# lpiccinelli-eth/UniDepth

Measured on NVIDIA H100. Metric: images/sec UniDepthV2.infer ViT-L/14 480x640, higher is better.
Workload: dtype f16 operands, f32 accumulate/residual

## Files before the change

unidepth_b200/csrc/gemm.cu:

```cuda
#include "common.h"
#include "ptx.cuh"

namespace udb {

constexpr int BM = 128;
constexpr int BK = 64;
constexpr int kEpiWarps = 8;
constexpr int kTP = 36;
constexpr int kThreads = (kEpiWarps + 4) * 32;

struct GemmArgs {
  int M, N, K, num_kb;
  int tiles_m, tiles_n;
  int a_mode;
  int conv_B, conv_H, conv_W, conv_cpb , conv_off, conv_TH, conv_TW, conv_tx, conv_ty;
  const float* bias;
  const float* gamma;
  const void* resid;
  int resid_f32;
  void* out;
  int out_f32;
  __half* out2;
  int out2_leaky;
  int act;
  int store_mode;
  long long ldc, ldr;
  int rpg, gstride, roff;
  int resid_mod, resid_roff;
  int ct_k, ct_cout, ct_h, ct_w, ct_pad;
  int conv_coff;
  const float* head_w;
  float head_b, head_add;
  int a_wrap;
  int out_split;
  float* stats_out;
  const float* ln_stats;
  const float* ln_c1;
  int ln_parts, ln_part_cols;
  float ln_eps;
};

template <int BN>
struct GemmCfg {
  static constexpr int kStages = BN >= 256 ? 3 : (BN >= 192 ? 4 : (BN >= 128 ? 5 : 7));
  static constexpr int kABytes = BM * BK * 2;
  static constexpr int kBBytes = BN * BK * 2;
  static constexpr int kStageBytes = kABytes + kBBytes;
  static constexpr int kStagingBytes = kEpiWarps * (32 * kTP * 4 + 2 * 32 * 4);
  static constexpr int kSmemBytes = kStages * kStageBytes + kStagingBytes + 256 ;
  static_assert(kSmemBytes <= 232448, "shared memory per block");
};

struct EpiWarp {
  float* T;
  float* Twg;
  uint32_t* roff_out;
  uint32_t* roff_res;
  int wg, wq, grp, lane, r_in_tile;
};

template <int BN, bool LNF>
__device__ __forceinline__ void epilogue_tile(const GemmArgs& p, const EpiWarp& w, const float (&acc)[BN / 2], const int mt,
                                              const int nt) {
  constexpr int kGroups = BN >= 64 ? 2 : 1;
  constexpr int kColsPerGrp = BN / kGroups;
  const int grp = w.grp, lane = w.lane, r_in_tile = w.r_in_tile;
  const bool active = grp < kGroups;
  float* T = w.T;
  uint32_t* roff_out = w.roff_out;
  uint32_t* roff_res = w.roff_res;
  bool valid = false;
  long long out_off = 0, res_off = 0;
  uint32_t vmask = 0;
  float ln_mean = 0.f, ln_rstd = 1.f;
  float st_pivot = 0.f, st_s1 = 0.f, st_s2 = 0.f;
  bool st_first = true;
  if (active) {

    const int m = mt * BM + r_in_tile;
    if (p.store_mode == UDB_STORE_CONVTILE || p.store_mode == UDB_STORE_HEAD) {
      const int per_img = p.conv_tx * p.conv_ty;
      const int b = mt / per_img;
      const int r = mt % per_img;
      const int y = (r / p.conv_tx) * p.conv_TH + r_in_tile / p.conv_TW;
      const int x = (r % p.conv_tx) * p.conv_TW + r_in_tile % p.conv_TW;
      valid = (b < p.conv_B) && (y < p.conv_H) && (x < p.conv_W);
      out_off = (((long long)b * p.conv_H + y) * p.conv_W + x) * p.ldc;
      res_off = (((long long)b * p.conv_H + y) * p.conv_W + x) * p.ldr;
    } else if (p.store_mode == UDB_STORE_CONVT) {
      valid = m < p.M;
      const int hw = p.ct_h * p.ct_w;
      const int b = m / hw;
      const int r = m % hw;
      const int y = r / p.ct_w, x = r % p.ct_w;
      const long long W2 = (long long)p.ct_w * p.ct_k + 2 * p.ct_pad;
      const long long H2 = (long long)p.ct_h * p.ct_k + 2 * p.ct_pad;
      out_off = ((b * H2 + (long long)y * p.ct_k + p.ct_pad) * W2 + (long long)x * p.ct_k + p.ct_pad) * p.ct_cout;
      res_off = out_off;
    } else {
      valid = m < p.M;
      long long orow = m;
      if (p.rpg > 0) orow = (long long)(m / p.rpg) * p.gstride + (m % p.rpg) + p.roff;
      out_off = orow * p.ldc;
      res_off = (p.resid_mod > 0) ? ((long long)(m % p.resid_mod) + p.resid_roff) * p.ldr
                                  : orow * p.ldr;
    }
    vmask = __ballot_sync(0xffffffffu, valid);
    roff_out[lane] = static_cast<uint32_t>(out_off);
    roff_res[lane] = static_cast<uint32_t>(res_off);
    __syncwarp();
    if (LNF && p.ln_stats) {
      const float2* sp = reinterpret_cast<const float2*>(p.ln_stats) + (long long)(valid ? m : 0) * p.ln_parts;
      float ms = 0.f, m2 = 0.f;
      for (int q = 0; q < p.ln_parts; ++q) ms += sp[q].x;
      ln_mean = ms / (float)p.ln_parts;
      for (int q = 0; q < p.ln_parts; ++q) {
        const float2 t = sp[q];
        m2 += t.y + (float)p.ln_part_cols * (t.x - ln_mean) * (t.x - ln_mean);
      }
      ln_rstd = rsqrtf(m2 / (float)(p.ln_parts * p.ln_part_cols) + p.ln_eps);
    }
  }
  const int frow = 16 * (w.wq & 1) + (lane >> 2), fcol = 2 * (lane & 3);
#pragma unroll
  for (int c = 0; c < kColsPerGrp; c += 32) {
    bar_sync(1 + w.wg, 128);
#pragma unroll
    for (int gi = 0; gi < kGroups; ++gi) {
      float* Tt = w.Twg + ((w.wq >> 1) | (gi << 1)) * 32 * kTP;
#pragma unroll
      for (int j = 0; j < 4; ++j) {
        const int f = ((gi * kColsPerGrp + c) / 8 + j) * 4;
        *reinterpret_cast<float2*>(Tt + frow * kTP + 8 * j + fcol) = make_float2(acc[f], acc[f + 1]);
        *reinterpret_cast<float2*>(Tt + (frow + 8) * kTP + 8 * j + fcol) = make_float2(acc[f + 2], acc[f + 3]);
      }
    }
    bar_sync(1 + w.wg, 128);
    if (!active) continue;
    const int col = grp * kColsPerGrp + c;
    const int n0 = nt * BN + col;
    float v[32];
#pragma unroll
    for (int j = 0; j < 32; j += 4) {
      const float4 t = *reinterpret_cast<const float4*>(T + lane * kTP + j);
      v[j] = t.x; v[j + 1] = t.y; v[j + 2] = t.z; v[j + 3] = t.w;
    }
    __syncwarp();
    if (n0 >= p.N) continue;
    if (LNF && p.ln_stats) {
      const float4* cp = reinterpret_cast<const float4*>(p.ln_c1 + n0);
      const float mr = ln_mean * ln_rstd;
#pragma unroll
      for (int j = 0; j < 8; ++j) {
        const float4 c4 = __ldg(cp + j);
        v[4 * j] = fmaf(v[4 * j], ln_rstd, -mr * c4.x);
        v[4 * j + 1] = fmaf(v[4 * j + 1], ln_rstd, -mr * c4.y);
        v[4 * j + 2] = fmaf(v[4 * j + 2], ln_rstd, -mr * c4.z);
        v[4 * j + 3] = fmaf(v[4 * j + 3], ln_rstd, -mr * c4.w);
      }
    }
    if (p.bias) {
      const float4* bp = reinterpret_cast<const float4*>(p.bias + n0);
#pragma unroll
      for (int j = 0; j < 8; ++j) {
        const float4 b4 = __ldg(bp + j);
        v[4 * j] += b4.x; v[4 * j + 1] += b4.y; v[4 * j + 2] += b4.z; v[4 * j + 3] += b4.w;
      }
    }
    if (p.act == UDB_ACT_GELU) {
#pragma unroll
      for (int j = 0; j < 32; j += 2) gelu_erf_pair(v[j], v[j + 1]);
    } else if (p.act == UDB_ACT_LEAKY) {
#pragma unroll
      for (int j = 0; j < 32; ++j) v[j] = leaky(v[j]);
    }
    if (p.store_mode == UDB_STORE_HEAD) {
      float head = p.head_b;
#pragma unroll
      for (int j = 0; j < 32; ++j) head = fmaf(v[j], __ldg(p.head_w + j), head);
      head = fminf(fmaxf(head, -8.0f), 8.0f) + p.head_add;
      if (valid) reinterpret_cast<float*>(p.out)[out_off] = expf(head);
      continue;
    }
    if (p.gamma) {
      const float4* gp = reinterpret_cast<const float4*>(p.gamma + n0);
#pragma unroll
      for (int j = 0; j < 8; ++j) {
        const float4 g4 = __ldg(gp + j);
        v[4 * j] *= g4.x; v[4 * j + 1] *= g4.y; v[4 * j + 2] *= g4.z; v[4 * j + 3] *= g4.w;
      }
    }
    long long coff = n0;
    if (p.store_mode == UDB_STORE_CONVT) {
      const int tap = n0 / p.ct_cout;
      const int co = n0 % p.ct_cout;
      const long long W2 = (long long)p.ct_w * p.ct_k + 2 * p.ct_pad;
      coff = ((long long)(tap / p.ct_k) * W2 + (tap % p.ct_k)) * p.ct_cout + co;
    }
    const uint32_t c32 = static_cast<uint32_t>(coff);
    const int l4 = (lane & 7) * 4, rq = lane >> 3;
    float* Trow = T + lane * kTP;
    auto stage_rows = [&](const float (&x)[32]) {
#pragma unroll
      for (int j = 0; j < 32; j += 4)
        *reinterpret_cast<float4*>(Trow + j) = make_float4(x[j], x[j + 1], x[j + 2], x[j + 3]);
    };
    auto for_rows = [&](auto&& body) {
      if (vmask == 0xffffffffu) {
#pragma unroll
        for (int i = 0; i < 8; ++i) body(4 * i + rq, true);
      } else {
#pragma unroll
        for (int i = 0; i < 8; ++i) body(4 * i + rq, ((vmask >> (4 * i + rq)) & 1u) != 0);
      }
    };
    if (p.resid) {
      if (p.resid_f32) {
        const float* rp = reinterpret_cast<const float*>(p.resid) + c32 + l4;
        float4 tmp[8];
        int k = 0;
        for_rows([&](int rr, bool ok) {
          tmp[k++] = ok ? *reinterpret_cast<const float4*>(rp + roff_res[rr]) : make_float4(0.f, 0.f, 0.f, 0.f);
        });
#pragma unroll
        for (int i = 0; i < 8; ++i) *reinterpret_cast<float4*>(T + (4 * i + rq) * kTP + l4) = tmp[i];
      } else {
        const __half* rp = reinterpret_cast<const __half*>(p.resid) + c32 + l4;
        uint2 tmp[8];
        int k = 0;
        for_rows([&](int rr, bool ok) {
          tmp[k++] = ok ? *reinterpret_cast<const uint2*>(rp + roff_res[rr]) : make_uint2(0u, 0u);
        });
#pragma unroll
        for (int i = 0; i < 8; ++i) {
          const float2 a = __half22float2(*reinterpret_cast<const __half2*>(&tmp[i].x));
          const float2 b = __half22float2(*reinterpret_cast<const __half2*>(&tmp[i].y));
          *reinterpret_cast<float4*>(T + (4 * i + rq) * kTP + l4) = make_float4(a.x, a.y, b.x, b.y);
        }
      }
      __syncwarp();
#pragma unroll
      for (int j = 0; j < 32; j += 4) {
        const float4 t = *reinterpret_cast<const float4*>(Trow + j);
        v[j] += t.x; v[j + 1] += t.y; v[j + 2] += t.z; v[j + 3] += t.w;
      }
      __syncwarp();
    }
    if (LNF && p.stats_out) {
      if (st_first) { st_pivot = v[0]; st_first = false; }
#pragma unroll
      for (int j = 0; j < 32; ++j) {
        const float dlt = v[j] - st_pivot;
        st_s1 += dlt;
        st_s2 = fmaf(dlt, dlt, st_s2);
      }
    }
    if (p.out) {
      stage_rows(v);
      __syncwarp();
      if (p.out_f32) {
        float* op = reinterpret_cast<float*>(p.out) + c32 + l4;
        for_rows([&](int rr, bool ok) {
          if (ok) *reinterpret_cast<float4*>(op + roff_out[rr]) = *reinterpret_cast<const float4*>(T + rr * kTP + l4);
        });
      } else {
        __half* op = reinterpret_cast<__half*>(p.out) + c32 + l4;
        if (p.out_split == 0) {
          for_rows([&](int rr, bool ok) {
            const float4 t = *reinterpret_cast<const float4*>(T + rr * kTP + l4);
            if (ok) *reinterpret_cast<uint2*>(op + roff_out[rr]) = make_uint2(pack_half2(t.x, t.y), pack_half2(t.z, t.w));
          });
        } else {
          for_rows([&](int rr, bool ok) {
            const float4 t = *reinterpret_cast<const float4*>(T + rr * kTP + l4);
            const uint2 hi = make_uint2(pack_half2(t.x, t.y), pack_half2(t.z, t.w));
            const float2 h01 = __half22float2(*reinterpret_cast<const __half2*>(&hi.x));
            const float2 h23 = __half22float2(*reinterpret_cast<const __half2*>(&hi.y));
            if (ok) {
              *reinterpret_cast<uint2*>(op + roff_out[rr]) = hi;
              *reinterpret_cast<uint2*>(op + roff_out[rr] + p.out_split) =
                  make_uint2(pack_half2(t.x - h01.x, t.y - h01.y), pack_half2(t.z - h23.x, t.w - h23.y));
            }
          });
        }
      }
      __syncwarp();
    }
    if (p.out2) {
      if (p.out2_leaky) {
#pragma unroll
        for (int j = 0; j < 32; ++j) v[j] = leaky(v[j]);
        stage_rows(v);
      } else if (!p.out) {
        stage_rows(v);
      }
      __syncwarp();
      __half* op = p.out2 + c32 + l4;
      for_rows([&](int rr, bool ok) {
        const float4 t = *reinterpret_cast<const float4*>(T + rr * kTP + l4);
        if (ok) *reinterpret_cast<uint2*>(op + roff_out[rr]) = make_uint2(pack_half2(t.x, t.y), pack_half2(t.z, t.w));
      });
      __syncwarp();
    }
  }
  if (LNF && p.stats_out && active && valid && !st_first) {
    const float n = (float)kColsPerGrp;
    const float mean_p = st_pivot + st_s1 / n;
    const float m2_p = fmaxf(st_s2 - st_s1 * st_s1 / n, 0.f);
    const long long orow = out_off / p.ldc;
    reinterpret_cast<float2*>(p.stats_out)[orow * (p.tiles_n * kGroups) + nt * kGroups + grp] = make_float2(mean_p, m2_p);
  }
}

template <int BN, bool LNF>
__global__ void __launch_bounds__(kThreads, 1)
gemm_f16_kernel(const __grid_constant__ CUtensorMap tmA, const __grid_constant__ CUtensorMap tmB,
                const GemmArgs p) {
  using Cfg = GemmCfg<BN>;
  constexpr int kStages = Cfg::kStages;
  extern __shared__ __align__(1024) uint8_t smem[];
  uint8_t* sA = smem;
  uint8_t* sB = smem + kStages * Cfg::kABytes;
  uint8_t* staging = smem + kStages * Cfg::kStageBytes;
  uint64_t* bars = reinterpret_cast<uint64_t*>(staging + Cfg::kStagingBytes);
  uint64_t* full_bar = bars;
  uint64_t* empty_bar = bars + kStages;

  const int warp = threadIdx.x >> 5;
  const int lane = threadIdx.x & 31;
  pdl_launch_dependents();

  if (threadIdx.x == 0) {
    if (smem_u32(smem) & 1023) __trap();
    prefetch_tmap(&tmA);
    prefetch_tmap(&tmB);
    for (int i = 0; i < kStages; ++i) {
      mbar_init(&full_bar[i], 1);
      mbar_init(&empty_bar[i], kEpiWarps);
    }
    fence_barrier_init();
  }
  __syncthreads();
  pdl_wait();

  const int num_tiles = p.tiles_m * p.tiles_n;

  if (warp >= kEpiWarps) {
    setmaxnreg_dec<40>();
    if (warp != kEpiWarps) return;
    const bool elected = elect_one();
    int stage = 0;
    uint32_t phase = 0;
    for (int tile = blockIdx.x; tile < num_tiles; tile += gridDim.x) {
      const int mt = tile / p.tiles_n;
      const int nt = tile % p.tiles_n;
      int cb = 0, cy = 0, cx = 0;
      if (p.a_mode == UDB_A_CONV3X3) {
        const int per_img = p.conv_tx * p.conv_ty;
        cb = mt / per_img;
        const int r = mt % per_img;
        cy = (r / p.conv_tx) * p.conv_TH + p.conv_off;
        cx = (r % p.conv_tx) * p.conv_TW + p.conv_off;
      }
      for (int kb = 0; kb < p.num_kb; ++kb) {
        mbar_wait(&empty_bar[stage], phase ^ 1);
        if (elected) {
          mbar_arrive_expect_tx(&full_bar[stage], Cfg::kStageBytes);
          if (p.a_mode == UDB_A_CONV3X3) {
            const int tap = kb / p.conv_cpb;
            const int c0 = p.conv_coff + (kb % p.conv_cpb) * BK;
            tma_load_4d(sA + stage * Cfg::kABytes, &tmA, &full_bar[stage], c0, cx + tap % 3, cy + tap / 3, cb);
          } else {
            int ka = kb * BK;
            if (p.a_wrap && ka >= p.a_wrap) ka -= p.a_wrap;
            tma_load_2d(sA + stage * Cfg::kABytes, &tmA, &full_bar[stage], ka, mt * BM);
          }
          tma_load_2d(sB + stage * Cfg::kBBytes, &tmB, &full_bar[stage], kb * BK, nt * BN);
        }
        __syncwarp();
        if (++stage == kStages) {
          stage = 0;
          phase ^= 1;
        }
      }
    }
  } else {
    setmaxnreg_inc<232>();
    const int wg = warp >> 2, wq = warp & 3;
    float* Twg = reinterpret_cast<float*>(staging) + wg * 4 * 32 * kTP;
    uint32_t* roff = reinterpret_cast<uint32_t*>(staging + kEpiWarps * 32 * kTP * 4) + warp * 64;
    const EpiWarp ctx{Twg + wq * 32 * kTP, Twg, roff, roff + 32, wg, wq, wq >> 1, lane, 64 * wg + 32 * (wq & 1) + lane};
    float acc[BN / 2];
#pragma unroll
    for (int i = 0; i < BN / 2; ++i) acc[i] = 0.f;
    int stage = 0;
    uint32_t phase = 0;
    for (int tile = blockIdx.x; tile < num_tiles; tile += gridDim.x) {
      const int mt = tile / p.tiles_n;
      const int nt = tile % p.tiles_n;
      int prev = -1;
      for (int kb = 0; kb < p.num_kb; ++kb) {
        mbar_wait(&full_bar[stage], phase);
        const uint64_t da = gmma_desc_sw128(smem_u32(sA + stage * Cfg::kABytes + wg * 64 * 128), 16, 1024);
        const uint64_t db = gmma_desc_sw128(smem_u32(sB + stage * Cfg::kBBytes), 16, 1024);
        wgmma_fence();
#pragma unroll
        for (int k = 0; k < BK / 16; ++k) WgmmaSS<BN>::run(acc, da + 2 * k, db + 2 * k, (kb | k) != 0 ? 1u : 0u);
        wgmma_commit();
        wgmma_wait<1>();
        if (prev >= 0 && lane == 0) mbar_arrive(&empty_bar[prev]);
        prev = stage;
        if (++stage == kStages) {
          stage = 0;
          phase ^= 1;
        }
      }
      wgmma_wait<0>();
      wgmma_fence_regs(acc);
      if (prev >= 0 && lane == 0) mbar_arrive(&empty_bar[prev]);
      epilogue_tile<BN, LNF>(p, ctx, acc, mt, nt);
    }
  }
}

template <int BN, bool LNF>
static int launch_gemm(const CUtensorMap& tmA, const CUtensorMap& tmB, const GemmArgs& a, cudaStream_t st) {
  using Cfg = GemmCfg<BN>;
  static std::atomic<uint64_t> attr_mask{0};
  if (first_on_device(attr_mask)) {
    cudaError_t e = cudaFuncSetAttribute(gemm_f16_kernel<BN, LNF>, cudaFuncAttributeMaxDynamicSharedMemorySize,
                                         Cfg::kSmemBytes);
    if (e != cudaSuccess) {
      set_error("gemm: cudaFuncSetAttribute(%d B smem): %s", Cfg::kSmemBytes, cudaGetErrorString(e));
      return 1;
    }
  }
  const int tiles = a.tiles_m * a.tiles_n;
  const int grid = tiles < num_sms() ? tiles : num_sms();
  cudaError_t e = launch_ex(gemm_f16_kernel<BN, LNF>, dim3(grid), dim3(kThreads), Cfg::kSmemBytes, st, 1, tmA, tmB, a);
  if (e != cudaSuccess) {
    set_error("gemm_f16_kernel launch: %s", cudaGetErrorString(e));
    return 1;
  }
  return check_launch("gemm_f16_kernel");
}

static bool aligned(const void* p, uintptr_t bytes) { return (reinterpret_cast<uintptr_t>(p) & (bytes - 1)) == 0; }

static int check_gemm_layout(const udb_gemm_t* g) {
  const int sm = g->store_mode;
  if (g->M < 1 || g->N < 1 || g->K < 1) { set_error("udb_gemm_f16: M=%d N=%d K=%d must be >= 1", g->M, g->N, g->K); return 1; }
  if (sm < UDB_STORE_ROWS || sm > UDB_STORE_HEAD) { set_error("udb_gemm_f16: unknown store_mode %d", sm); return 1; }
  const long long ldr = g->ldr > 0 ? g->ldr : g->ldc;
  if (sm == UDB_STORE_HEAD) {
    if (!g->out || !g->out_f32 || !aligned(g->out, 4)) { set_error("udb_gemm_f16: HEAD store needs a 4-byte aligned f32 `out`"); return 1; }
    if (!g->head_w || !aligned(g->head_w, 16)) { set_error("udb_gemm_f16: `head_w` must be non-null and 16-byte aligned"); return 1; }
  } else {
    if (g->out && !aligned(g->out, g->out_f32 ? 16 : 8)) {
      set_error("udb_gemm_f16: `out` %p must be %d-byte aligned", g->out, g->out_f32 ? 16 : 8); return 1;
    }
    if (g->out2 && !aligned(g->out2, 8)) { set_error("udb_gemm_f16: `out2` %p must be 8-byte aligned", g->out2); return 1; }
    if (g->resid && !aligned(g->resid, g->resid_f32 ? 16 : 8)) {
      set_error("udb_gemm_f16: `resid` %p must be %d-byte aligned", g->resid, g->resid_f32 ? 16 : 8); return 1;
    }
    if (sm != UDB_STORE_CONVT) {
      if ((g->out || g->out2) && (g->ldc < 1 || g->ldc % 4)) { set_error("udb_gemm_f16: `ldc`=%lld must be a positive multiple of 4", (long long)g->ldc); return 1; }
      if (g->resid && (ldr < 1 || ldr % 4)) { set_error("udb_gemm_f16: `ldr`=%lld must be a positive multiple of 4", ldr); return 1; }
      if ((g->out || g->out2) && g->ldc < (long long)g->N + g->out_split) {
        set_error("udb_gemm_f16: `ldc`=%lld < N + out_split = %lld: rows would overlap", (long long)g->ldc, (long long)g->N + g->out_split);
        return 1;
      }
      if (g->resid && ldr < g->N) { set_error("udb_gemm_f16: `ldr`=%lld < N=%d: residual rows would overlap", ldr, g->N); return 1; }
    }
  }
  if (g->out_split < 0 || g->out_split % 4) { set_error("udb_gemm_f16: `out_split`=%d must be a non-negative multiple of 4", g->out_split); return 1; }
  if (!aligned(g->bias, 16)) { set_error("udb_gemm_f16: `bias` %p must be 16-byte aligned", (const void*)g->bias); return 1; }
  if (!aligned(g->gamma, 16)) { set_error("udb_gemm_f16: `gamma` %p must be 16-byte aligned", (const void*)g->gamma); return 1; }
  if (!aligned(g->ln_c1, 16)) { set_error("udb_gemm_f16: `ln_c1` %p must be 16-byte aligned", (const void*)g->ln_c1); return 1; }
  if (!aligned(g->ln_stats_out, 8) || !aligned(g->ln_stats_in, 8)) { set_error("udb_gemm_f16: `ln_stats_*` must be 8-byte aligned"); return 1; }

  long long out_row = 0, res_row = 0;
  if (sm == UDB_STORE_ROWS) {
    const int m = g->M - 1;
    long long orow = m;
    if (g->rows_per_group > 0) {
      if (g->group_stride < 0 || g->row_offset < 0) {
        set_error("udb_gemm_f16: `group_stride`=%d and `row_offset`=%d must be >= 0", g->group_stride, g->row_offset); return 1;
      }
      const long long rpg = g->rows_per_group, grp = m / rpg;
      orow = grp * g->group_stride + m % rpg + g->row_offset;
      if (grp > 0 && (grp - 1) * g->group_stride + rpg - 1 + g->row_offset > orow) orow = (grp - 1) * g->group_stride + rpg - 1 + g->row_offset;
    }
    long long rrow = orow;
    if (g->resid_mod > 0) {
      if (g->resid_row_offset < 0) { set_error("udb_gemm_f16: `resid_row_offset`=%d must be >= 0", g->resid_row_offset); return 1; }
      rrow = (long long)(g->resid_mod < g->M ? g->resid_mod : g->M) - 1 + g->resid_row_offset;
    }
    out_row = orow * g->ldc;
    res_row = rrow * ldr;
  } else if (sm == UDB_STORE_CONVT) {
    if (g->ct_k < 1 || g->ct_h < 1 || g->ct_w < 1 || g->ct_pad < 0 || g->ct_cout < 1) {
      set_error("udb_gemm_f16: CONVT geometry `ct_k`=%d `ct_h`=%d `ct_w`=%d `ct_pad`=%d `ct_cout`=%d", g->ct_k, g->ct_h, g->ct_w, g->ct_pad,
                g->ct_cout);
      return 1;
    }
    if (g->N != g->ct_k * g->ct_k * g->ct_cout) { set_error("udb_gemm_f16: CONVT needs N == ct_k^2 * ct_cout (N=%d)", g->N); return 1; }
    const long long m = g->M - 1, hw = (long long)g->ct_h * g->ct_w, b = m / hw, r = m % hw, y = r / g->ct_w, x = r % g->ct_w;
    const long long W2 = (long long)g->ct_w * g->ct_k + 2 * g->ct_pad, H2 = (long long)g->ct_h * g->ct_k + 2 * g->ct_pad;
    out_row = res_row = ((b * H2 + y * g->ct_k + g->ct_pad) * W2 + x * g->ct_k + g->ct_pad) * g->ct_cout;
  } else {
    if (g->conv_B < 1 || g->conv_H < 1 || g->conv_W < 1) {
      set_error("udb_gemm_f16: conv_B=%d conv_H=%d conv_W=%d must be >= 1", g->conv_B, g->conv_H, g->conv_W); return 1;
    }
    const long long last_px = (long long)g->conv_B * g->conv_H * g->conv_W - 1;
    out_row = last_px * g->ldc;
    res_row = last_px * ldr;
  }
  const long long lim = 1ll << 32;
  if ((g->out || g->out2) && out_row >= lim) { set_error("udb_gemm_f16: `out` row offset %lld exceeds 2^32 elements", out_row); return 1; }
  if (g->resid && res_row >= lim) { set_error("udb_gemm_f16: `resid` row offset %lld exceeds 2^32 elements", res_row); return 1; }

  if (g->a_mode == UDB_A_CONV3X3) {
    const int pad = g->conv_off == 0 ? 2 : (g->conv_off == -1 ? 0 : -1);
    if (pad < 0) { set_error("udb_gemm_f16: `conv_off`=%d must be 0 (prepadded) or -1 (zero padding)", g->conv_off); return 1; }
    if (g->conv_inH != g->conv_H + pad || g->conv_inW != g->conv_W + pad) {
      set_error("udb_gemm_f16: `conv_inH`x`conv_inW` = %dx%d must be %dx%d for conv_off %d", g->conv_inH, g->conv_inW, g->conv_H + pad,
                g->conv_W + pad, g->conv_off);
      return 1;
    }
  }
  return 0;
}

}

extern "C" int udb_gemm_f16(const udb_gemm_t* g, void* stream) {
  using namespace udb;
  if (!g || !g->a || !g->w) { set_error("udb_gemm_f16: null operand"); return 1; }
  if (g->N % 32 != 0) { set_error("udb_gemm_f16: N=%d must be a multiple of 32", g->N); return 1; }
  if (check_gemm_layout(g)) return 1;
  GemmArgs a{};
  a.M = g->M; a.N = g->N; a.K = g->K;
  a.num_kb = (g->K + BK - 1) / BK;
  a.a_mode = g->a_mode;
  a.bias = g->bias; a.gamma = g->gamma; a.resid = g->resid; a.resid_f32 = g->resid_f32;
  a.out = g->out; a.out_f32 = g->out_f32; a.out2 = reinterpret_cast<__half*>(g->out2); a.out2_leaky = g->out2_leaky;
  a.act = g->act; a.store_mode = g->store_mode;
  a.ldc = g->ldc; a.ldr = g->ldr > 0 ? g->ldr : g->ldc;
  a.rpg = g->rows_per_group; a.gstride = g->group_stride; a.roff = g->row_offset;
  a.resid_mod = g->resid_mod; a.resid_roff = g->resid_row_offset;
  a.ct_k = g->ct_k; a.ct_cout = g->ct_cout; a.ct_h = g->ct_h; a.ct_w = g->ct_w; a.ct_pad = g->ct_pad;
  a.conv_coff = g->conv_coff;
  a.head_w = g->head_w; a.head_b = g->head_b; a.head_add = g->head_add;
  a.a_wrap = 0;
  a.out_split = g->out_split;
  if (g->a_split_k > 0) {
    if (g->a_mode != UDB_A_MATRIX || g->a_split_k % BK || g->K != 3 * g->a_split_k || g->lda < 2 * g->a_split_k) {
      set_error("udb_gemm_f16: split operands need a_mode MATRIX, K1 %% 64 == 0, K == 3*K1, lda >= 2*K1 (K1=%d K=%d lda=%d)",
                g->a_split_k, g->K, g->lda);
      return 1;
    }
    a.a_wrap = 2 * g->a_split_k;
  }
  a.stats_out = g->ln_stats_out; a.ln_stats = g->ln_stats_in; a.ln_c1 = g->ln_c1; a.ln_eps = g->ln_eps;
  a.ln_parts = g->ln_parts; a.ln_part_cols = g->ln_part_cols;
  if ((g->ln_stats_out || g->ln_stats_in) && g->store_mode != UDB_STORE_ROWS) {
    set_error("udb_gemm_f16: fused LayerNorm statistics need the ROWS store"); return 1;
  }
  if (g->ln_stats_in && (!g->ln_c1 || g->ln_parts <= 0 || g->ln_part_cols <= 0 || g->rows_per_group > 0)) {
    set_error("udb_gemm_f16: ln_stats_in needs ln_c1, ln_parts, ln_part_cols and an identity row map"); return 1;
  }
  if (g->out_split && (g->out_f32 || !g->out || g->store_mode != UDB_STORE_ROWS)) {
    set_error("udb_gemm_f16: out_split needs an f16 `out` with the ROWS store"); return 1;
  }

  int bn;
  if (g->store_mode == UDB_STORE_HEAD) {
    if (g->N != 32) { set_error("udb_gemm_f16: HEAD store needs N == 32"); return 1; }
    bn = 32;
  } else if (g->N % 256 == 0) bn = 256;
  else if (g->N % 192 == 0) bn = 192;
  else if (g->N % 128 == 0) bn = 128;
  else if (g->N % 64 == 0) bn = 64;
  else bn = 32;
  if (g->store_mode == UDB_STORE_CONVT && (g->ct_cout % 32) != 0) {
    set_error("udb_gemm_f16: CONVT needs Cout %% 32 == 0"); return 1;
  }
  a.tiles_n = (g->N + bn - 1) / bn;
  if (g->ln_stats_out) {
    const int groups = bn >= 64 ? 2 : 1;
    if (g->N % bn || g->ln_parts != a.tiles_n * groups || g->ln_part_cols != bn / groups) {
      set_error("udb_gemm_f16: ln_stats_out with N=%d runs as %d parts of %d columns (caller said %d x %d)", g->N, a.tiles_n * groups,
                bn / groups, g->ln_parts, g->ln_part_cols);
      return 1;
    }
  }

  CUtensorMap tmA, tmB;
  if (g->a_mode == UDB_A_CONV3X3) {
    if (g->conv_C % BK != 0 || g->K != 9 * g->conv_C) {
      set_error("udb_gemm_f16: conv3x3 needs C %% 64 == 0 and K == 9*C (C=%d K=%d)", g->conv_C, g->K);
      return 1;
    }
    if (g->store_mode != UDB_STORE_CONVTILE && g->store_mode != UDB_STORE_HEAD) {
      set_error("udb_gemm_f16: conv3x3 operand needs a CONVTILE or HEAD store"); return 1;
    }
    const int TH = g->conv_TH > 0 ? g->conv_TH : 8, TW = g->conv_TW > 0 ? g->conv_TW : 16;
    if (TH * TW != BM) { set_error("udb_gemm_f16: conv tile %dx%d != 128 pixels", TH, TW); return 1; }
    a.conv_B = g->conv_B; a.conv_H = g->conv_H; a.conv_W = g->conv_W; a.conv_cpb = g->conv_C / BK; a.conv_off = g->conv_off;
    a.conv_TH = TH; a.conv_TW = TW;
    a.conv_tx = (g->conv_W + TW - 1) / TW; a.conv_ty = (g->conv_H + TH - 1) / TH;
    a.tiles_m = g->conv_B * a.conv_tx * a.conv_ty;
    a.M = a.tiles_m * BM;
    const uint64_t cs = g->conv_cstride > 0 ? g->conv_cstride : g->conv_C;
    if ((uint64_t)g->conv_coff + g->conv_C > cs || (g->conv_coff % 8)) {
      set_error("udb_gemm_f16: bad conv channel slice (off %d, C %d, stride %d)", g->conv_coff, g->conv_C, (int)cs);
      return 1;
    }
    const uint64_t dims[4] = {cs, (uint64_t)g->conv_inW, (uint64_t)g->conv_inH, (uint64_t)g->conv_B};
    const uint64_t str[3] = {cs * 2, (uint64_t)g->conv_inW * cs * 2, (uint64_t)g->conv_inH * g->conv_inW * cs * 2};
    const uint32_t box[4] = {(uint32_t)BK, (uint32_t)TW, (uint32_t)TH, 1};
    if (make_tmap_f16(&tmA, g->a, 4, dims, str, box, true)) return 1;
  } else {
    a.tiles_m = (g->M + BM - 1) / BM;
    if (g->store_mode == UDB_STORE_CONVTILE || g->store_mode == UDB_STORE_HEAD) {
      set_error("udb_gemm_f16: tile store modes need a_mode == CONV3X3"); return 1;
    }
    const uint64_t dims[2] = {(uint64_t)(g->a_split_k > 0 ? 2 * g->a_split_k : g->K), (uint64_t)g->M};
    const uint64_t str[1] = {(uint64_t)g->lda * 2};
    const uint32_t box[2] = {(uint32_t)BK, (uint32_t)BM};
    if (make_tmap_f16(&tmA, g->a, 2, dims, str, box, true)) return 1;
  }
  {
    const uint64_t dims[2] = {(uint64_t)g->K, (uint64_t)g->N};
    const uint64_t str[1] = {(uint64_t)g->ldw * 2};
    const uint32_t box[2] = {(uint32_t)BK, (uint32_t)bn};
    if (make_tmap_f16(&tmB, g->w, 2, dims, str, box, true)) return 1;
  }
  cudaStream_t st = reinterpret_cast<cudaStream_t>(stream);
  note_work(2.0 * a.M * (double)g->N * g->K,
            2.0 * ((double)a.M * (g->a_mode == UDB_A_CONV3X3 ? g->conv_C : (g->a_split_k ? 2 * g->a_split_k : g->K)) + (double)g->N * g->K) +
                (double)a.M * g->N * ((g->out ? (g->out_f32 ? 4 : 2) : 0) + (g->out2 ? 2 : 0) + (g->resid ? (g->resid_f32 ? 4 : 2) : 0)));
  const bool lnf = g->ln_stats_out || g->ln_stats_in;
  if (lnf) {
    switch (bn) {
      case 256: return launch_gemm<256, true>(tmA, tmB, a, st);
      case 192: return launch_gemm<192, true>(tmA, tmB, a, st);
      case 128: return launch_gemm<128, true>(tmA, tmB, a, st);
      case 64: return launch_gemm<64, true>(tmA, tmB, a, st);
      default: return launch_gemm<32, true>(tmA, tmB, a, st);
    }
  }
  switch (bn) {
    case 256: return launch_gemm<256, false>(tmA, tmB, a, st);
    case 192: return launch_gemm<192, false>(tmA, tmB, a, st);
    case 128: return launch_gemm<128, false>(tmA, tmB, a, st);
    case 64: return launch_gemm<64, false>(tmA, tmB, a, st);
    default: return launch_gemm<32, false>(tmA, tmB, a, st);
  }
}
```

unidepth_b200/csrc/ptx.cuh:

```cuda
#pragma once
#include <cuda_fp16.h>
#include <cuda_runtime.h>
#include <stdint.h>
#include <stdio.h>

namespace udb {

__device__ __forceinline__ uint32_t smem_u32(const void* p) {
  return static_cast<uint32_t>(__cvta_generic_to_shared(p));
}

__device__ __forceinline__ bool elect_one() {
  uint32_t pred = 0;
  asm volatile(
      "{\n\t"
      ".reg .b32 rx;\n\t"
      ".reg .pred px;\n\t"
      "elect.sync rx|px, 0xffffffff;\n\t"
      "selp.b32 %0, 1, 0, px;\n\t"
      "}\n"
      : "=r"(pred));
  return pred != 0;
}

__device__ __forceinline__ void pdl_launch_dependents() {
  asm volatile("griddepcontrol.launch_dependents;" ::: "memory");
}
__device__ __forceinline__ void pdl_wait() { asm volatile("griddepcontrol.wait;" ::: "memory"); }

__device__ __forceinline__ void mbar_init(uint64_t* bar, uint32_t count) {
  asm volatile("mbarrier.init.shared::cta.b64 [%0], %1;" ::"r"(smem_u32(bar)), "r"(count));
}
__device__ __forceinline__ void fence_barrier_init() {
  asm volatile("fence.mbarrier_init.release.cluster;" ::: "memory");
}
__device__ __forceinline__ void mbar_arrive(uint64_t* bar) {
  asm volatile("mbarrier.arrive.shared::cta.b64 _, [%0];" ::"r"(smem_u32(bar)) : "memory");
}
__device__ __forceinline__ void mbar_arrive_expect_tx(uint64_t* bar, uint32_t bytes) {
  asm volatile("mbarrier.arrive.expect_tx.shared::cta.b64 _, [%0], %1;" ::"r"(smem_u32(bar)),
               "r"(bytes)
               : "memory");
}
__device__ __forceinline__ bool mbar_try_wait(uint64_t* bar, uint32_t parity) {
  uint32_t ok;
  asm volatile(
      "{\n\t"
      ".reg .pred p;\n\t"
      "mbarrier.try_wait.parity.shared::cta.b64 p, [%1], %2, %3;\n\t"
      "selp.b32 %0, 1, 0, p;\n\t"
      "}\n"
      : "=r"(ok)
      : "r"(smem_u32(bar)), "r"(parity), "r"(20000u)
      : "memory");
  return ok != 0;
}
#ifndef UDB_SPIN_LIMIT
#define UDB_SPIN_LIMIT (1u << 22)
#endif
__device__ __forceinline__ void mbar_wait(uint64_t* bar, uint32_t parity) {
  if (mbar_try_wait(bar, parity)) return;
  uint32_t spins = 0;
  while (!mbar_try_wait(bar, parity)) {
    if (++spins > UDB_SPIN_LIMIT) __trap();
  }
}

__device__ __forceinline__ void fence_proxy_async_smem() {
  asm volatile("fence.proxy.async.shared::cta;" ::: "memory");
}

__device__ __forceinline__ void prefetch_tmap(const void* tmap) {
  asm volatile("prefetch.tensormap [%0];" ::"l"(reinterpret_cast<uint64_t>(tmap)) : "memory");
}
__device__ __forceinline__ void tma_load_2d(void* smem_dst, const void* tmap, uint64_t* bar, int c0,
                                            int c1) {
  asm volatile(
      "cp.async.bulk.tensor.2d.shared::cluster.global.mbarrier::complete_tx::bytes"
      " [%0], [%1, {%3, %4}], [%2];" ::"r"(smem_u32(smem_dst)),
      "l"(reinterpret_cast<uint64_t>(tmap)), "r"(smem_u32(bar)), "r"(c0), "r"(c1)
      : "memory");
}
__device__ __forceinline__ void tma_load_3d(void* smem_dst, const void* tmap, uint64_t* bar, int c0,
                                            int c1, int c2) {
  asm volatile(
      "cp.async.bulk.tensor.3d.shared::cluster.global.mbarrier::complete_tx::bytes"
      " [%0], [%1, {%3, %4, %5}], [%2];" ::"r"(smem_u32(smem_dst)),
      "l"(reinterpret_cast<uint64_t>(tmap)), "r"(smem_u32(bar)), "r"(c0), "r"(c1), "r"(c2)
      : "memory");
}
__device__ __forceinline__ void tma_load_4d(void* smem_dst, const void* tmap, uint64_t* bar, int c0,
                                            int c1, int c2, int c3) {
  asm volatile(
      "cp.async.bulk.tensor.4d.shared::cluster.global.mbarrier::complete_tx::bytes"
      " [%0], [%1, {%3, %4, %5, %6}], [%2];" ::"r"(smem_u32(smem_dst)),
      "l"(reinterpret_cast<uint64_t>(tmap)), "r"(smem_u32(bar)), "r"(c0), "r"(c1), "r"(c2), "r"(c3)
      : "memory");
}


__device__ __forceinline__ void wgmma_fence() { asm volatile("wgmma.fence.sync.aligned;" ::: "memory"); }
__device__ __forceinline__ void wgmma_commit() { asm volatile("wgmma.commit_group.sync.aligned;" ::: "memory"); }
template <int N>
__device__ __forceinline__ void wgmma_wait() {
  asm volatile("wgmma.wait_group.sync.aligned %0;" ::"n"(N) : "memory");
}
template <int R>
__device__ __forceinline__ void wgmma_fence_regs(float (&d)[R]) {
#pragma unroll
  for (int i = 0; i < R; ++i) asm volatile("" : "+f"(d[i])::"memory");
}
template <uint32_t R>
__device__ __forceinline__ void setmaxnreg_inc() { asm volatile("setmaxnreg.inc.sync.aligned.u32 %0;" ::"n"(R)); }
template <uint32_t R>
__device__ __forceinline__ void setmaxnreg_dec() { asm volatile("setmaxnreg.dec.sync.aligned.u32 %0;" ::"n"(R)); }
__device__ __forceinline__ void bar_sync(int id, int threads) {
  asm volatile("bar.sync %0, %1;" ::"r"(id), "r"(threads) : "memory");
}

__device__ __forceinline__ uint64_t gmma_desc_sw128(uint32_t smem_addr, uint32_t lbo_bytes, uint32_t sbo_bytes) {
  uint64_t d = 0;
  d |= static_cast<uint64_t>((smem_addr & 0x3FFFF) >> 4);
  d |= static_cast<uint64_t>((lbo_bytes >> 4) & 0x3FFF) << 16;
  d |= static_cast<uint64_t>((sbo_bytes >> 4) & 0x3FFF) << 32;
  d |= static_cast<uint64_t>(1) << 62;
  return d;
}

__device__ __forceinline__ void wgmma_ss_n32(float (&d)[16], uint64_t da, uint64_t db, uint32_t scale_d) {
  asm volatile(
      "{\n\t.reg .pred p;\n\tsetp.ne.b32 p, %18, 0;\n\t"
      "wgmma.mma_async.sync.aligned.m64n32k16.f32.f16.f16 {%0, %1, %2, %3, %4, %5, %6, %7, %8, %9, %10, %11, %12, %13, %14, %15}, %16, %17, p, 1, 1, 0, 0;\n\t}\n"
      : "+f"(d[0]), "+f"(d[1]), "+f"(d[2]), "+f"(d[3]), "+f"(d[4]), "+f"(d[5]), "+f"(d[6]), "+f"(d[7]), "+f"(d[8]), "+f"(d[9]), "+f"(d[10]), "+f"(d[11]), "+f"(d[12]), "+f"(d[13]), "+f"(d[14]), "+f"(d[15])
      : "l"(da), "l"(db), "r"(scale_d));
}
__device__ __forceinline__ void wgmma_ss_n64(float (&d)[32], uint64_t da, uint64_t db, uint32_t scale_d) {
  asm volatile(
      "{\n\t.reg .pred p;\n\tsetp.ne.b32 p, %34, 0;\n\t"
      "wgmma.mma_async.sync.aligned.m64n64k16.f32.f16.f16 {%0, %1, %2, %3, %4, %5, %6, %7, %8, %9, %10, %11, %12, %13, %14, %15, %16, %17, %18, %19, %20, %21, %22, %23, %24, %25, %26, %27, %28, %29, %30, %31}, %32, %33, p, 1, 1, 0, 0;\n\t}\n"
      : "+f"(d[0]), "+f"(d[1]), "+f"(d[2]), "+f"(d[3]), "+f"(d[4]), "+f"(d[5]), "+f"(d[6]), "+f"(d[7]), "+f"(d[8]), "+f"(d[9]), "+f"(d[10]), "+f"(d[11]), "+f"(d[12]), "+f"(d[13]), "+f"(d[14]), "+f"(d[15]), "+f"(d[16]), "+f"(d[17]), "+f"(d[18]), "+f"(d[19]), "+f"(d[20]), "+f"(d[21]), "+f"(d[22]), "+f"(d[23]), "+f"(d[24]), "+f"(d[25]), "+f"(d[26]), "+f"(d[27]), "+f"(d[28]), "+f"(d[29]), "+f"(d[30]), "+f"(d[31])
      : "l"(da), "l"(db), "r"(scale_d));
}
__device__ __forceinline__ void wgmma_ss_n128(float (&d)[64], uint64_t da, uint64_t db, uint32_t scale_d) {
  asm volatile(
      "{\n\t.reg .pred p;\n\tsetp.ne.b32 p, %66, 0;\n\t"
      "wgmma.mma_async.sync.aligned.m64n128k16.f32.f16.f16 {%0, %1, %2, %3, %4, %5, %6, %7, %8, %9, %10, %11, %12, %13, %14, %15, %16, %17, %18, %19, %20, %21, %22, %23, %24, %25, %26, %27, %28, %29, %30, %31, %32, %33, %34, %35, %36, %37, %38, %39, %40, %41, %42, %43, %44, %45, %46, %47, %48, %49, %50, %51, %52, %53, %54, %55, %56, %57, %58, %59, %60, %61, %62, %63}, %64, %65, p, 1, 1, 0, 0;\n\t}\n"
      : "+f"(d[0]), "+f"(d[1]), "+f"(d[2]), "+f"(d[3]), "+f"(d[4]), "+f"(d[5]), "+f"(d[6]), "+f"(d[7]), "+f"(d[8]), "+f"(d[9]), "+f"(d[10]), "+f"(d[11]), "+f"(d[12]), "+f"(d[13]), "+f"(d[14]), "+f"(d[15]), "+f"(d[16]), "+f"(d[17]), "+f"(d[18]), "+f"(d[19]), "+f"(d[20]), "+f"(d[21]), "+f"(d[22]), "+f"(d[23]), "+f"(d[24]), "+f"(d[25]), "+f"(d[26]), "+f"(d[27]), "+f"(d[28]), "+f"(d[29]), "+f"(d[30]), "+f"(d[31]), "+f"(d[32]), "+f"(d[33]), "+f"(d[34]), "+f"(d[35]), "+f"(d[36]), "+f"(d[37]), "+f"(d[38]), "+f"(d[39]), "+f"(d[40]), "+f"(d[41]), "+f"(d[42]), "+f"(d[43]), "+f"(d[44]), "+f"(d[45]), "+f"(d[46]), "+f"(d[47]), "+f"(d[48]), "+f"(d[49]), "+f"(d[50]), "+f"(d[51]), "+f"(d[52]), "+f"(d[53]), "+f"(d[54]), "+f"(d[55]), "+f"(d[56]), "+f"(d[57]), "+f"(d[58]), "+f"(d[59]), "+f"(d[60]), "+f"(d[61]), "+f"(d[62]), "+f"(d[63])
      : "l"(da), "l"(db), "r"(scale_d));
}
__device__ __forceinline__ void wgmma_ss_n192(float (&d)[96], uint64_t da, uint64_t db, uint32_t scale_d) {
  asm volatile(
      "{\n\t.reg .pred p;\n\tsetp.ne.b32 p, %98, 0;\n\t"
      "wgmma.mma_async.sync.aligned.m64n192k16.f32.f16.f16 {%0, %1, %2, %3, %4, %5, %6, %7, %8, %9, %10, %11, %12, %13, %14, %15, %16, %17, %18, %19, %20, %21, %22, %23, %24, %25, %26, %27, %28, %29, %30, %31, %32, %33, %34, %35, %36, %37, %38, %39, %40, %41, %42, %43, %44, %45, %46, %47, %48, %49, %50, %51, %52, %53, %54, %55, %56, %57, %58, %59, %60, %61, %62, %63, %64, %65, %66, %67, %68, %69, %70, %71, %72, %73, %74, %75, %76, %77, %78, %79, %80, %81, %82, %83, %84, %85, %86, %87, %88, %89, %90, %91, %92, %93, %94, %95}, %96, %97, p, 1, 1, 0, 0;\n\t}\n"
      : "+f"(d[0]), "+f"(d[1]), "+f"(d[2]), "+f"(d[3]), "+f"(d[4]), "+f"(d[5]), "+f"(d[6]), "+f"(d[7]), "+f"(d[8]), "+f"(d[9]), "+f"(d[10]), "+f"(d[11]), "+f"(d[12]), "+f"(d[13]), "+f"(d[14]), "+f"(d[15]), "+f"(d[16]), "+f"(d[17]), "+f"(d[18]), "+f"(d[19]), "+f"(d[20]), "+f"(d[21]), "+f"(d[22]), "+f"(d[23]), "+f"(d[24]), "+f"(d[25]), "+f"(d[26]), "+f"(d[27]), "+f"(d[28]), "+f"(d[29]), "+f"(d[30]), "+f"(d[31]), "+f"(d[32]), "+f"(d[33]), "+f"(d[34]), "+f"(d[35]), "+f"(d[36]), "+f"(d[37]), "+f"(d[38]), "+f"(d[39]), "+f"(d[40]), "+f"(d[41]), "+f"(d[42]), "+f"(d[43]), "+f"(d[44]), "+f"(d[45]), "+f"(d[46]), "+f"(d[47]), "+f"(d[48]), "+f"(d[49]), "+f"(d[50]), "+f"(d[51]), "+f"(d[52]), "+f"(d[53]), "+f"(d[54]), "+f"(d[55]), "+f"(d[56]), "+f"(d[57]), "+f"(d[58]), "+f"(d[59]), "+f"(d[60]), "+f"(d[61]), "+f"(d[62]), "+f"(d[63]), "+f"(d[64]), "+f"(d[65]), "+f"(d[66]), "+f"(d[67]), "+f"(d[68]), "+f"(d[69]), "+f"(d[70]), "+f"(d[71]), "+f"(d[72]), "+f"(d[73]), "+f"(d[74]), "+f"(d[75]), "+f"(d[76]), "+f"(d[77]), "+f"(d[78]), "+f"(d[79]), "+f"(d[80]), "+f"(d[81]), "+f"(d[82]), "+f"(d[83]), "+f"(d[84]), "+f"(d[85]), "+f"(d[86]), "+f"(d[87]), "+f"(d[88]), "+f"(d[89]), "+f"(d[90]), "+f"(d[91]), "+f"(d[92]), "+f"(d[93]), "+f"(d[94]), "+f"(d[95])
      : "l"(da), "l"(db), "r"(scale_d));
}
__device__ __forceinline__ void wgmma_ss_n256(float (&d)[128], uint64_t da, uint64_t db, uint32_t scale_d) {
  asm volatile(
      "{\n\t.reg .pred p;\n\tsetp.ne.b32 p, %130, 0;\n\t"
      "wgmma.mma_async.sync.aligned.m64n256k16.f32.f16.f16 {%0, %1, %2, %3, %4, %5, %6, %7, %8, %9, %10, %11, %12, %13, %14, %15, %16, %17, %18, %19, %20, %21, %22, %23, %24, %25, %26, %27, %28, %29, %30, %31, %32, %33, %34, %35, %36, %37, %38, %39, %40, %41, %42, %43, %44, %45, %46, %47, %48, %49, %50, %51, %52, %53, %54, %55, %56, %57, %58, %59, %60, %61, %62, %63, %64, %65, %66, %67, %68, %69, %70, %71, %72, %73, %74, %75, %76, %77, %78, %79, %80, %81, %82, %83, %84, %85, %86, %87, %88, %89, %90, %91, %92, %93, %94, %95, %96, %97, %98, %99, %100, %101, %102, %103, %104, %105, %106, %107, %108, %109, %110, %111, %112, %113, %114, %115, %116, %117, %118, %119, %120, %121, %122, %123, %124, %125, %126, %127}, %128, %129, p, 1, 1, 0, 0;\n\t}\n"
      : "+f"(d[0]), "+f"(d[1]), "+f"(d[2]), "+f"(d[3]), "+f"(d[4]), "+f"(d[5]), "+f"(d[6]), "+f"(d[7]), "+f"(d[8]), "+f"(d[9]), "+f"(d[10]), "+f"(d[11]), "+f"(d[12]), "+f"(d[13]), "+f"(d[14]), "+f"(d[15]), "+f"(d[16]), "+f"(d[17]), "+f"(d[18]), "+f"(d[19]), "+f"(d[20]), "+f"(d[21]), "+f"(d[22]), "+f"(d[23]), "+f"(d[24]), "+f"(d[25]), "+f"(d[26]), "+f"(d[27]), "+f"(d[28]), "+f"(d[29]), "+f"(d[30]), "+f"(d[31]), "+f"(d[32]), "+f"(d[33]), "+f"(d[34]), "+f"(d[35]), "+f"(d[36]), "+f"(d[37]), "+f"(d[38]), "+f"(d[39]), "+f"(d[40]), "+f"(d[41]), "+f"(d[42]), "+f"(d[43]), "+f"(d[44]), "+f"(d[45]), "+f"(d[46]), "+f"(d[47]), "+f"(d[48]), "+f"(d[49]), "+f"(d[50]), "+f"(d[51]), "+f"(d[52]), "+f"(d[53]), "+f"(d[54]), "+f"(d[55]), "+f"(d[56]), "+f"(d[57]), "+f"(d[58]), "+f"(d[59]), "+f"(d[60]), "+f"(d[61]), "+f"(d[62]), "+f"(d[63]), "+f"(d[64]), "+f"(d[65]), "+f"(d[66]), "+f"(d[67]), "+f"(d[68]), "+f"(d[69]), "+f"(d[70]), "+f"(d[71]), "+f"(d[72]), "+f"(d[73]), "+f"(d[74]), "+f"(d[75]), "+f"(d[76]), "+f"(d[77]), "+f"(d[78]), "+f"(d[79]), "+f"(d[80]), "+f"(d[81]), "+f"(d[82]), "+f"(d[83]), "+f"(d[84]), "+f"(d[85]), "+f"(d[86]), "+f"(d[87]), "+f"(d[88]), "+f"(d[89]), "+f"(d[90]), "+f"(d[91]), "+f"(d[92]), "+f"(d[93]), "+f"(d[94]), "+f"(d[95]), "+f"(d[96]), "+f"(d[97]), "+f"(d[98]), "+f"(d[99]), "+f"(d[100]), "+f"(d[101]), "+f"(d[102]), "+f"(d[103]), "+f"(d[104]), "+f"(d[105]), "+f"(d[106]), "+f"(d[107]), "+f"(d[108]), "+f"(d[109]), "+f"(d[110]), "+f"(d[111]), "+f"(d[112]), "+f"(d[113]), "+f"(d[114]), "+f"(d[115]), "+f"(d[116]), "+f"(d[117]), "+f"(d[118]), "+f"(d[119]), "+f"(d[120]), "+f"(d[121]), "+f"(d[122]), "+f"(d[123]), "+f"(d[124]), "+f"(d[125]), "+f"(d[126]), "+f"(d[127])
      : "l"(da), "l"(db), "r"(scale_d));
}
__device__ __forceinline__ void wgmma_rs_n64_tb(float (&d)[32], const uint32_t (&a)[4], uint64_t db, uint32_t scale_d) {
  asm volatile(
      "{\n\t.reg .pred p;\n\tsetp.ne.b32 p, %37, 0;\n\t"
      "wgmma.mma_async.sync.aligned.m64n64k16.f32.f16.f16 {%0, %1, %2, %3, %4, %5, %6, %7, %8, %9, %10, %11, %12, %13, %14, %15, %16, %17, %18, %19, %20, %21, %22, %23, %24, %25, %26, %27, %28, %29, %30, %31}, {%32, %33, %34, %35}, %36, p, 1, 1, 1;\n\t}\n"
      : "+f"(d[0]), "+f"(d[1]), "+f"(d[2]), "+f"(d[3]), "+f"(d[4]), "+f"(d[5]), "+f"(d[6]), "+f"(d[7]), "+f"(d[8]), "+f"(d[9]), "+f"(d[10]), "+f"(d[11]), "+f"(d[12]), "+f"(d[13]), "+f"(d[14]), "+f"(d[15]), "+f"(d[16]), "+f"(d[17]), "+f"(d[18]), "+f"(d[19]), "+f"(d[20]), "+f"(d[21]), "+f"(d[22]), "+f"(d[23]), "+f"(d[24]), "+f"(d[25]), "+f"(d[26]), "+f"(d[27]), "+f"(d[28]), "+f"(d[29]), "+f"(d[30]), "+f"(d[31])
      : "r"(a[0]), "r"(a[1]), "r"(a[2]), "r"(a[3]), "l"(db), "r"(scale_d));
}

template <int N> struct WgmmaSS;
template <> struct WgmmaSS<32> { static __device__ __forceinline__ void run(float (&d)[16], uint64_t a, uint64_t b, uint32_t s) { wgmma_ss_n32(d, a, b, s); } };
template <> struct WgmmaSS<64> { static __device__ __forceinline__ void run(float (&d)[32], uint64_t a, uint64_t b, uint32_t s) { wgmma_ss_n64(d, a, b, s); } };
template <> struct WgmmaSS<128> { static __device__ __forceinline__ void run(float (&d)[64], uint64_t a, uint64_t b, uint32_t s) { wgmma_ss_n128(d, a, b, s); } };
template <> struct WgmmaSS<192> { static __device__ __forceinline__ void run(float (&d)[96], uint64_t a, uint64_t b, uint32_t s) { wgmma_ss_n192(d, a, b, s); } };
template <> struct WgmmaSS<256> { static __device__ __forceinline__ void run(float (&d)[128], uint64_t a, uint64_t b, uint32_t s) { wgmma_ss_n256(d, a, b, s); } };

__device__ __forceinline__ uint64_t pack2(float lo, float hi) {
  uint64_t d;
  asm("mov.b64 %0, {%1, %2};" : "=l"(d) : "f"(lo), "f"(hi));
  return d;
}
__device__ __forceinline__ uint64_t pack2u(uint32_t lo, uint32_t hi) {
  uint64_t d;
  asm("mov.b64 %0, {%1, %2};" : "=l"(d) : "r"(lo), "r"(hi));
  return d;
}
__device__ __forceinline__ void unpack2(uint64_t v, float& lo, float& hi) {
  asm("mov.b64 {%0, %1}, %2;" : "=f"(lo), "=f"(hi) : "l"(v));
}
__device__ __forceinline__ uint64_t fma2(uint64_t a, uint64_t b, uint64_t c) {
  float a0, a1, b0, b1, c0, c1;
  unpack2(a, a0, a1);
  unpack2(b, b0, b1);
  unpack2(c, c0, c1);
  return pack2(fmaf(a0, b0, c0), fmaf(a1, b1, c1));
}
__device__ __forceinline__ uint64_t mul2(uint64_t a, uint64_t b) {
  float a0, a1, b0, b1;
  unpack2(a, a0, a1);
  unpack2(b, b0, b1);
  return pack2(__fmul_rn(a0, b0), __fmul_rn(a1, b1));
}

__device__ __forceinline__ float gelu_erf(float x) {
  return 0.5f * x * (1.0f + erff(x * 0.70710678118654752440f));
}
__device__ __forceinline__ float gelu_erf_fast(float x) {
  const float z = fabsf(x) * 0.70710678118654752440f;
  float t;
  asm("rcp.approx.ftz.f32 %0, %1;" : "=f"(t) : "f"(fmaf(0.3275911f, z, 1.0f)));
  float poly = fmaf(t, 1.061405429f, -1.453152027f);
  poly = fmaf(poly, t, 1.421413741f);
  poly = fmaf(poly, t, -0.284496736f);
  poly = fmaf(poly, t, 0.254829592f);
  poly *= t;
  float e;
  asm("ex2.approx.ftz.f32 %0, %1;" : "=f"(e) : "f"(z * z * -1.4426950408889634f));
  const float erf_abs = fmaf(-poly, e, 1.0f);
  const float h = 0.5f * x;
  return fmaf(copysignf(erf_abs, x), h, h);
}
__device__ __forceinline__ void gelu_erf_pair(float& x0, float& x1) {
  const float z0 = fabsf(x0) * 0.70710678118654752440f, z1 = fabsf(x1) * 0.70710678118654752440f;
  const uint64_t z = pack2(z0, z1);
  uint64_t q = fma2(z, pack2(0.0000430638f, 0.0000430638f), pack2(0.0002765672f, 0.0002765672f));
  q = fma2(q, z, pack2(0.0001520143f, 0.0001520143f));
  q = fma2(q, z, pack2(0.0092705272f, 0.0092705272f));
  q = fma2(q, z, pack2(0.0422820123f, 0.0422820123f));
  q = fma2(q, z, pack2(0.0705230784f, 0.0705230784f));
  q = fma2(q, z, pack2(1.0f, 1.0f));
  q = mul2(q, q);
  q = mul2(q, q);
  q = mul2(q, q);
  q = mul2(q, q);
  float p0, p1, r0, r1;
  unpack2(q, p0, p1);
  asm("rcp.approx.ftz.f32 %0, %1;" : "=f"(r0) : "f"(p0));
  asm("rcp.approx.ftz.f32 %0, %1;" : "=f"(r1) : "f"(p1));
  const float h0 = 0.5f * x0, h1 = 0.5f * x1;
  x0 = fmaf(copysignf(1.0f - r0, x0), h0, h0);
  x1 = fmaf(copysignf(1.0f - r1, x1), h1, h1);
}
__device__ __forceinline__ float leaky(float x) { return x > 0.f ? x : 0.01f * x; }

__device__ __forceinline__ uint32_t pack_half2(float a, float b) {
  __half2 h = __floats2half2_rn(a, b);
  return *reinterpret_cast<uint32_t*>(&h);
}

}
```

Baseline: 215.9.

## Pair CTAs in 2-CTA clusters and multicast weight tiles via TMA

Launches the GEMM as 2-CTA clusters in which both CTAs share an N tile but work on adjacent M tiles. Each CTA loads half of the B (weight) tile and multicasts it to both CTAs, so each weight tile is fetched from L2 once per pair instead of twice. Empty barriers now count arrivals from both CTAs, consumers signal the peer's barrier remotely, and a cluster barrier is added at start and end. The grid is sized from cudaOccupancyMaxActiveClusters. In exchange, the two CTAs progress in lockstep, odd tiles_m leaves one CTA computing a padding tile, and cluster placement may leave some SMs unused.

Result: no change. 216.3 (median of 6 runs) (+0.2%).

```diff
diff --git a/unidepth_b200/csrc/gemm.cu b/unidepth_b200/csrc/gemm.cu
--- a/unidepth_b200/csrc/gemm.cu
+++ b/unidepth_b200/csrc/gemm.cu
@@ -328,6 +328,7 @@
 
   const int warp = threadIdx.x >> 5;
   const int lane = threadIdx.x & 31;
+  const uint32_t rank = cluster_ctarank();
   pdl_launch_dependents();
 
   if (threadIdx.x == 0) {
@@ -336,51 +337,54 @@
     prefetch_tmap(&tmB);
     for (int i = 0; i < kStages; ++i) {
       mbar_init(&full_bar[i], 1);
-      mbar_init(&empty_bar[i], kEpiWarps);
+      mbar_init(&empty_bar[i], 2 * kEpiWarps);
     }
     fence_barrier_init();
   }
-  __syncthreads();
+  cluster_sync();
   pdl_wait();
 
-  const int num_tiles = p.tiles_m * p.tiles_n;
+  const int num_pairs = ((p.tiles_m + 1) / 2) * p.tiles_n;
+  const int cluster = blockIdx.x / 2, num_clusters = gridDim.x / 2;
 
   if (warp >= kEpiWarps) {
     setmaxnreg_dec<40>();
-    if (warp != kEpiWarps) return;
-    const bool elected = elect_one();
-    int stage = 0;
-    uint32_t phase = 0;
-    for (int tile = blockIdx.x; tile < num_tiles; tile += gridDim.x) {
-      const int mt = tile / p.tiles_n;
-      const int nt = tile % p.tiles_n;
-      int cb = 0, cy = 0, cx = 0;
-      if (p.a_mode == UDB_A_CONV3X3) {
-        const int per_img = p.conv_tx * p.conv_ty;
-        cb = mt / per_img;
-        const int r = mt % per_img;
-        cy = (r / p.conv_tx) * p.conv_TH + p.conv_off;
-        cx = (r % p.conv_tx) * p.conv_TW + p.conv_off;
-      }
-      for (int kb = 0; kb < p.num_kb; ++kb) {
-        mbar_wait(&empty_bar[stage], phase ^ 1);
-        if (elected) {
-          mbar_arrive_expect_tx(&full_bar[stage], Cfg::kStageBytes);
-          if (p.a_mode == UDB_A_CONV3X3) {
-            const int tap = kb / p.conv_cpb;
-            const int c0 = p.conv_coff + (kb % p.conv_cpb) * BK;
-            tma_load_4d(sA + stage * Cfg::kABytes, &tmA, &full_bar[stage], c0, cx + tap % 3, cy + tap / 3, cb);
-          } else {
-            int ka = kb * BK;
-            if (p.a_wrap && ka >= p.a_wrap) ka -= p.a_wrap;
-            tma_load_2d(sA + stage * Cfg::kABytes, &tmA, &full_bar[stage], ka, mt * BM);
+    if (warp == kEpiWarps) {
+      const bool elected = elect_one();
+      int stage = 0;
+      uint32_t phase = 0;
+      for (int q = cluster; q < num_pairs; q += num_clusters) {
+        const int mt = 2 * (q / p.tiles_n) + rank;
+        const int nt = q % p.tiles_n;
+        int cb = 0, cy = 0, cx = 0;
+        if (p.a_mode == UDB_A_CONV3X3) {
+          const int per_img = p.conv_tx * p.conv_ty;
+          cb = mt / per_img;
+          const int r = mt % per_img;
+          cy = (r / p.conv_tx) * p.conv_TH + p.conv_off;
+          cx = (r % p.conv_tx) * p.conv_TW + p.conv_off;
+        }
+        for (int kb = 0; kb < p.num_kb; ++kb) {
+          mbar_wait(&empty_bar[stage], phase ^ 1);
+          if (elected) {
+            mbar_arrive_expect_tx(&full_bar[stage], Cfg::kStageBytes);
+            if (p.a_mode == UDB_A_CONV3X3) {
+              const int tap = kb / p.conv_cpb;
+              const int c0 = p.conv_coff + (kb % p.conv_cpb) * BK;
+              tma_load_4d(sA + stage * Cfg::kABytes, &tmA, &full_bar[stage], c0, cx + tap % 3, cy + tap / 3, cb);
+            } else {
+              int ka = kb * BK;
+              if (p.a_wrap && ka >= p.a_wrap) ka -= p.a_wrap;
+              tma_load_2d(sA + stage * Cfg::kABytes, &tmA, &full_bar[stage], ka, mt * BM);
+            }
+            tma_load_2d_multicast(sB + stage * Cfg::kBBytes + rank * (Cfg::kBBytes / 2), &tmB, &full_bar[stage], 0x3,
+                                  kb * BK, nt * BN + rank * (BN / 2));
           }
-          tma_load_2d(sB + stage * Cfg::kBBytes, &tmB, &full_bar[stage], kb * BK, nt * BN);
-        }
-        __syncwarp();
-        if (++stage == kStages) {
-          stage = 0;
-          phase ^= 1;
+          __syncwarp();
+          if (++stage == kStages) {
+            stage = 0;
+            phase ^= 1;
+          }
         }
       }
     }
@@ -393,11 +397,16 @@
     float acc[BN / 2];
 #pragma unroll
     for (int i = 0; i < BN / 2; ++i) acc[i] = 0.f;
+    const uint32_t peer_empty_bar = mapa_shared(smem_u32(empty_bar), rank ^ 1);
+    auto release = [&](int s) {
+      mbar_arrive(&empty_bar[s]);
+      mbar_arrive_cluster(peer_empty_bar + 8 * s);
+    };
     int stage = 0;
     uint32_t phase = 0;
-    for (int tile = blockIdx.x; tile < num_tiles; tile += gridDim.x) {
-      const int mt = tile / p.tiles_n;
-      const int nt = tile % p.tiles_n;
+    for (int q = cluster; q < num_pairs; q += num_clusters) {
+      const int mt = 2 * (q / p.tiles_n) + rank;
+      const int nt = q % p.tiles_n;
       int prev = -1;
       for (int kb = 0; kb < p.num_kb; ++kb) {
         mbar_wait(&full_bar[stage], phase);
@@ -408,7 +417,7 @@
         for (int k = 0; k < BK / 16; ++k) WgmmaSS<BN>::run(acc, da + 2 * k, db + 2 * k, (kb | k) != 0 ? 1u : 0u);
         wgmma_commit();
         wgmma_wait<1>();
-        if (prev >= 0 && lane == 0) mbar_arrive(&empty_bar[prev]);
+        if (prev >= 0 && lane == 0) release(prev);
         prev = stage;
         if (++stage == kStages) {
           stage = 0;
@@ -417,10 +426,11 @@
       }
       wgmma_wait<0>();
       wgmma_fence_regs(acc);
-      if (prev >= 0 && lane == 0) mbar_arrive(&empty_bar[prev]);
+      if (prev >= 0 && lane == 0) release(prev);
       epilogue_tile<BN, LNF>(p, ctx, acc, mt, nt);
     }
   }
+  cluster_sync();
 }
 
 template <int BN, bool LNF>
@@ -435,9 +445,32 @@
       return 1;
     }
   }
-  const int tiles = a.tiles_m * a.tiles_n;
-  const int grid = tiles < num_sms() ? tiles : num_sms();
-  cudaError_t e = launch_ex(gemm_f16_kernel<BN, LNF>, dim3(grid), dim3(kThreads), Cfg::kSmemBytes, st, 1, tmA, tmB, a);
+  static std::atomic<int> max_clusters[64];
+  int dev = 0;
+  cudaGetDevice(&dev);
+  int clusters = max_clusters[dev & 63].load(std::memory_order_relaxed);
+  if (clusters == 0) {
+    cudaLaunchConfig_t cfg{};
+    cudaLaunchAttribute attr{};
+    attr.id = cudaLaunchAttributeClusterDimension;
+    attr.val.clusterDim.x = 2;
+    attr.val.clusterDim.y = 1;
+    attr.val.clusterDim.z = 1;
+    cfg.gridDim = dim3(2 * (num_sms() / 2));
+    cfg.blockDim = dim3(kThreads);
+    cfg.dynamicSmemBytes = Cfg::kSmemBytes;
+    cfg.attrs = &attr;
+    cfg.numAttrs = 1;
+    cudaError_t e = cudaOccupancyMaxActiveClusters(&clusters, gemm_f16_kernel<BN, LNF>, &cfg);
+    if (e != cudaSuccess || clusters < 1) {
+      set_error("gemm: cudaOccupancyMaxActiveClusters: %s (%d clusters)", cudaGetErrorString(e), clusters);
+      return 1;
+    }
+    max_clusters[dev & 63].store(clusters, std::memory_order_relaxed);
+  }
+  const int pairs = ((a.tiles_m + 1) / 2) * a.tiles_n;
+  if (pairs < clusters) clusters = pairs;
+  cudaError_t e = launch_ex(gemm_f16_kernel<BN, LNF>, dim3(2 * clusters), dim3(kThreads), Cfg::kSmemBytes, st, 2, tmA, tmB, a);
   if (e != cudaSuccess) {
     set_error("gemm_f16_kernel launch: %s", cudaGetErrorString(e));
     return 1;
@@ -634,7 +667,7 @@
   {
     const uint64_t dims[2] = {(uint64_t)g->K, (uint64_t)g->N};
     const uint64_t str[1] = {(uint64_t)g->ldw * 2};
-    const uint32_t box[2] = {(uint32_t)BK, (uint32_t)bn};
+    const uint32_t box[2] = {(uint32_t)BK, (uint32_t)bn / 2};
     if (make_tmap_f16(&tmB, g->w, 2, dims, str, box, true)) return 1;
   }
   cudaStream_t st = reinterpret_cast<cudaStream_t>(stream);
diff --git a/unidepth_b200/csrc/ptx.cuh b/unidepth_b200/csrc/ptx.cuh
--- a/unidepth_b200/csrc/ptx.cuh
+++ b/unidepth_b200/csrc/ptx.cuh
@@ -96,6 +96,31 @@
       " [%0], [%1, {%3, %4, %5, %6}], [%2];" ::"r"(smem_u32(smem_dst)),
       "l"(reinterpret_cast<uint64_t>(tmap)), "r"(smem_u32(bar)), "r"(c0), "r"(c1), "r"(c2), "r"(c3)
       : "memory");
+}
+__device__ __forceinline__ void tma_load_2d_multicast(void* smem_dst, const void* tmap, uint64_t* bar, uint16_t cta_mask,
+                                                      int c0, int c1) {
+  asm volatile(
+      "cp.async.bulk.tensor.2d.shared::cluster.global.mbarrier::complete_tx::bytes.multicast::cluster"
+      " [%0], [%1, {%4, %5}], [%2], %3;" ::"r"(smem_u32(smem_dst)),
+      "l"(reinterpret_cast<uint64_t>(tmap)), "r"(smem_u32(bar)), "h"(cta_mask), "r"(c0), "r"(c1)
+      : "memory");
+}
+
+__device__ __forceinline__ uint32_t cluster_ctarank() {
+  uint32_t r;
+  asm("mov.u32 %0, %%cluster_ctarank;" : "=r"(r));
+  return r;
+}
+__device__ __forceinline__ void cluster_sync() {
+  asm volatile("barrier.cluster.arrive.release.aligned;\n\tbarrier.cluster.wait.acquire.aligned;" ::: "memory");
+}
+__device__ __forceinline__ uint32_t mapa_shared(uint32_t addr, uint32_t cta) {
+  uint32_t r;
+  asm("mapa.shared::cluster.u32 %0, %1, %2;" : "=r"(r) : "r"(addr), "r"(cta));
+  return r;
+}
+__device__ __forceinline__ void mbar_arrive_cluster(uint32_t cluster_addr) {
+  asm volatile("mbarrier.arrive.shared::cluster.b64 _, [%0];" ::"r"(cluster_addr) : "memory");
 }
 
 
```
